# IBM/text-generation-inference

Measured on AMD Instinct MI355X. Metric: decode tokens/sec (Llama-7B int4 GPTQ, batch 32, ctx 1024) + p50 step latency, higher is better.
Workload: dtype f16

## Files before the change

### include/tgis_hip.h

```cpp
#ifndef TGIS_HIP_H
#define TGIS_HIP_H

#include <stdint.h>

#ifdef __cplusplus
extern "C" {
#endif

#define TGIS_OK 0
#define TGIS_EINVAL (-1)
#define TGIS_EHIP (-2)
#define TGIS_EUNSUPPORTED (-3)
#define TGIS_ENOMEM (-4)

#define TGIS_F16 0
#define TGIS_BF16 1

#define TGIS_KV_PAGE_TOKENS 32

#define TGIS_KV_MODEL 0
#define TGIS_KV_FP8_E4M3 1

const char* tgis_version(void);
const char* tgis_arch(void);
// ... 91 lines not shown
                             void* res_out, int64_t rows, int64_t hidden, float eps, int dtype, void* stream);
int tgis_layernorm2_residual_partial(const void* residual, const void* a, const float* a_slabs, int a_num_slabs,
                                     int64_t a_slab_ld, const void* a_bias, const void* b, const float* b_slabs,
                                     int b_num_slabs, int64_t b_slab_ld, const void* b_bias, const void* w1, const void* b1,
                                     const void* w2, const void* b2, void* y1, void* y2, void* res_out, int64_t rows,
                                     int64_t hidden, float eps, int dtype, void* stream);

int tgis_rope_kv_write(void* qkv, int64_t ld_qkv, const void* cos, const void* sin,
                       const int32_t* positions, const int32_t* slots, void* k_pool, void* v_pool,
                       int64_t T, int H, int Hkv, int D, int rot_dim, int dtype, void* stream);

int tgis_rope_kv_write_partial(const float* slabs, int num_slabs, int64_t slab_ld, const void* bias, void* qkv_out,
                               int64_t ld_qkv, const void* cos, const void* sin, const int32_t* positions,
                               const int32_t* slots, void* k_pool, void* v_pool, int64_t T, int H, int Hkv, int D,
                               int rot_dim, int dtype, void* stream);

int tgis_rope_kv_write_prefill(void* qkv, int64_t ld_qkv, const void* cos, const void* sin, const int32_t* positions,
                               const int32_t* cu_seqlens, const int32_t* block_tables, int64_t max_pages, void* k_pool,
                               void* v_pool, int64_t B, int64_t T, int64_t max_len, int H, int Hkv, int D, int rot_dim,
                               int dtype, void* stream);

int tgis_rope_kv_write_kv8(void* qkv, int64_t ld_qkv, const void* cos, const void* sin, const int32_t* positions,
                           const int32_t* slots, void* k_pool, void* v_pool, int64_t T, int H, int Hkv, int D, int rot_dim,
                           int dtype, void* stream, int kv_dtype, float k_scale, float v_scale);
int tgis_rope_kv_write_partial_kv8(const float* slabs, int num_slabs, int64_t slab_ld, const void* bias, void* qkv_out,
                                   int64_t ld_qkv, const void* cos, const void* sin, const int32_t* positions,
                                   const int32_t* slots, void* k_pool, void* v_pool, int64_t T, int H, int Hkv, int D,
                                   int rot_dim, int dtype, void* stream, int kv_dtype, float k_scale, float v_scale);
int tgis_rope_kv_write_prefill_kv8(void* qkv, int64_t ld_qkv, const void* cos, const void* sin, const int32_t* positions,
                                   const int32_t* cu_seqlens, const int32_t* block_tables, int64_t max_pages, void* k_pool,
                                   void* v_pool, int64_t B, int64_t T, int64_t max_len, int H, int Hkv, int D, int rot_dim,
                                   int dtype, void* stream, int kv_dtype, float k_scale, float v_scale);

int tgis_attn_num_splits(int64_t B, int Hkv, int H, int64_t max_q_len, int64_t max_ctx);
int64_t tgis_attn_workspace_bytes(int64_t total_q_tokens, int H, int Hkv, int D, int num_splits);
int tgis_attn_paged(const void* q, int64_t ld_q, const void* k_pool, const void* v_pool,
                    const int32_t* block_tables, int64_t max_pages, const int32_t* ctx_lens,
                    const int32_t* cu_seqlens_q, void* out, int64_t ld_out, int64_t B, int H, int Hkv, int D,
                    int64_t max_q_len, int64_t max_ctx, float scale, int dtype, int num_splits,
                    void* workspace, int64_t workspace_bytes, void* stream);
int tgis_attn_paged_kv8(const void* q, int64_t ld_q, const void* k_pool, const void* v_pool, const int32_t* block_tables,
                        int64_t max_pages, const int32_t* ctx_lens, const int32_t* cu_seqlens_q, void* out, int64_t ld_out,
                        int64_t B, int H, int Hkv, int D, int64_t max_q_len, int64_t max_ctx, float scale, int dtype,
                        int num_splits, void* workspace, int64_t workspace_bytes, void* stream, int kv_dtype,
                        float k_scale, float v_scale);

int tgis_act_mul(const void* gate_up, void* out, int64_t T, int64_t I, int act, int dtype, void* stream);
int tgis_gelu(const void* x, void* out, int64_t n, int tanh_approx, int dtype, void* stream);
int tgis_embedding(const int64_t* ids, const void* table, const int32_t* positions,
                   const void* pos_table, void* out, int64_t T, int64_t E, int64_t vocab_rows,
                   int64_t id_offset, int dtype, void* stream);
int tgis_decode_slots(const int32_t* positions, const int32_t* block_tables, int64_t max_pages,
                      int32_t* slots, int32_t* ctx_lens, int64_t B, void* stream);
int tgis_decode_advance(const int64_t* ids, int64_t* ids_copy, int64_t* position_ids, int64_t* all_input_ids,
                        int64_t ld_all, int32_t* cu_seqlens, const int32_t* cu_seqlens_q, int64_t* stage_ids,
                        int32_t* stage_positions, int64_t B, void* stream);

int64_t tgis_argmax_scratch_bytes(int64_t B);
int tgis_argmax_logprob(const void* logits, int64_t ld, int64_t B, int64_t V, int logits_f32, int dtype,
                        int64_t* ids_out, float* logprob_out, void* scratch, int64_t scratch_bytes, void* stream);

int tgis_warp_sample(const float* logits, int64_t ld_logits, float* scores, int64_t ld_scores, int64_t B,
                     int64_t V, const float* temperature, const int* top_k, const float* top_p_cut,
                     const float* typical_p, const float* rep_penalty, const int64_t* input_ids,
                     int64_t ld_ids, int64_t L, int64_t exclude_id, const float* eos_adjust, int64_t eos_id,
                     const int* do_sample, uint64_t* rng, int64_t* next_ids, float* next_logprob, float* lse,
                     void* stream);

#ifdef __cplusplus
}
#endif
#endif
```

### text-generation-inference_amd/csrc/norm.hip

```cpp
#include "common.h"
#include "dispatch.h"
#include "rowwise_plan.h"

namespace {

constexpr int MAX_HIDDEN = 16384;

template <int NT>
__device__ __forceinline__ float block_sum(float v, float* sh) {
    v = wave_sum(v);
    const int lane = threadIdx.x & 63, w = threadIdx.x >> 6;
    __syncthreads();
    if (lane == 0) sh[w] = v;
    __syncthreads();
    float t = 0.f;
#pragma unroll
    for (int k = 0; k < NT / 64; ++k) t += sh[k];
    return t;
}

template <typename T, bool RMS, bool PARTIAL, int NT>
__global__ __launch_bounds__(NT) void norm_kernel(const T* x, const T* residual,
                                                  const T* __restrict__ weight, const T* __restrict__ bias,
                                                  T* y, T* res_out, int hidden,
// ... 40 lines not shown
            V8 o;
            if (rr) {
#pragma unroll
                for (int e = 0; e < 8; ++e) v[it][e] = to_f32(a[e]) + to_f32(b[e]);
            } else {
#pragma unroll
                for (int e = 0; e < 8; ++e) v[it][e] = to_f32(a[e]);
            }
#pragma unroll
            for (int e = 0; e < 8; ++e) {
                o[e] = from_f32<T>(v[it][e]);
                s1 += v[it][e];
                s2 += v[it][e] * v[it][e];
            }
            if (res_out) st16(res_out + row * hidden + c * 8, o);
        }
    }
    float mean = 0.f, rstd;
    if (RMS) {
        float tot = block_sum<NT>(s2, sh);
        rstd = rsqrtf(tot / hidden + eps);
    } else {
        mean = block_sum<NT>(s1, sh) / hidden;
        float d2 = 0.f;
#pragma unroll
        for (int it = 0; it < MAXV; ++it) {
            int c = threadIdx.x + it * NT;
            if (c < nchunk) {
#pragma unroll
                for (int e = 0; e < 8; ++e) {
                    float d = v[it][e] - mean;
                    d2 += d * d;
                }
            }
        }
        float var = block_sum<NT>(d2, sh) / hidden;
        rstd = rsqrtf(var + eps);
    }
#pragma unroll
    for (int it = 0; it < MAXV; ++it) {
        int c = threadIdx.x + it * NT;
        if (c < nchunk) {
            const V8 wv = wvs[it];
            V8 o;
            if (bias) {
                const V8 bv = bvs[it];
#pragma unroll
                for (int e = 0; e < 8; ++e)
                    o[e] = from_f32<T>((v[it][e] - mean) * rstd * to_f32(wv[e]) + to_f32(bv[e]));
            } else {
#pragma unroll
                for (int e = 0; e < 8; ++e) o[e] = from_f32<T>((v[it][e] - mean) * rstd * to_f32(wv[e]));
            }
            st16(y + (y_frag ? xf_off(row, c * 8, hidden) : row * hidden + c * 8), o);
        }
    }
}

template <bool RMS>
static int launch_norm(const void* x, const void* residual, const void* weight, const void* bias, void* y,
                       void* res_out, int64_t rows, int64_t hidden, float eps, int dtype, void* stream,
                       const float* slabs = nullptr, int S = 0, int64_t slab_ld = 0, const void* xbias = nullptr,
                       int64_t ldy = 0) {
    TGIS_CHECK_ARG((x || slabs) && weight && y, "norm: null tensor");
    TGIS_CHECK_ARG(!slabs || (S >= 1 && slab_ld >= hidden && slab_ld % 4 == 0),
                   "norm: partial input needs a slab row stride >= hidden");
    TGIS_CHECK_ARG(hidden > 0 && hidden % 8 == 0 && hidden <= MAX_HIDDEN,
                   "norm: hidden (%ld) must be a multiple of 8 and <= %d", (long)hidden, MAX_HIDDEN);
    TGIS_CHECK_ARG(dtype == TGIS_F16 || dtype == TGIS_BF16, "norm: bad dtype");
    const int y_frag = ldy == TGIS_LD_FRAGMENTS;
    TGIS_CHECK_ARG(ldy == 0 || ldy == hidden || (y_frag && RMS && rows <= 64 && hidden % 64 == 0),
                   "norm: y is [rows, hidden] contiguous (ldy = 0 or hidden), or — RMSNorm, rows <= 64, hidden %% 64 == 0 — in "
                   "fragment order (ldy = TGIS_LD_FRAGMENTS)");
    if (rows == 0) return TGIS_OK;
    hipStream_t st = (hipStream_t)stream;
    TgisTimedScope timed(TGIS_OP_NORM, st);
    const bool wide = choose_norm(rows, hidden).nt == 512;
    return by_dtype(dtype, [&](auto t) {
        using T = type_of<decltype(t)>;
        return by_bool(slabs != nullptr, [&](auto partial) {
            return by_bool(wide, [&](auto w) {
                constexpr int NT = decltype(w)::value ? 512 : 256;
                hipLaunchKernelGGL((norm_kernel<T, RMS, decltype(partial)::value, NT>), dim3((unsigned)rows), dim3(NT), 0,
                                   st, (const T*)x, (const T*)residual, (const T*)weight, (const T*)bias, (T*)y,
                                   (T*)res_out, (int)hidden, eps, slabs, S, slab_ld, (const T*)xbias, y_frag);
                TGIS_CHECK_LAUNCH();
                return TGIS_OK;
            });
        });
    });
}

struct Addend {
    const void* x;
    const float* slabs;
    int S;
    int64_t slab_ld;
    const void* bias;
};

template <typename T>
__device__ __forceinline__ void add_addend(float (&v)[8], const Addend& ad, int64_t row, int hidden, int c) {
    using V8 = typename VecT<T>::x8;
    if (ad.slabs) {
        f32x4 lo, hi;
        sum_slabs8(ad.slabs + ((row >> 5) * ad.S * 32 + (row & 31)) * ad.slab_ld + c * 8, 32 * ad.slab_ld, ad.S, lo, hi);
// ... 87 lines not shown
                const V8 wb = ld16<V8>(w2 + c * 8), bb = ld16<V8>(b2 + c * 8);
#pragma unroll
                for (int e = 0; e < 8; ++e) o[e] = from_f32<T>(n[e] * to_f32(wb[e]) + to_f32(bb[e]));
                st16(y2 + row * hidden + c * 8, o);
            }
        }
    }
}

static int launch_layernorm2(const void* h, const Addend& A, const Addend& B, const void* w1, const void* b1,
                             const void* w2, const void* b2, void* y1, void* y2, void* res_out, int64_t rows,
                             int64_t hidden, float eps, int dtype, void* stream) {
    TGIS_CHECK_ARG(h && w1 && b1 && y1, "tgis_layernorm2_residual: null tensor");
    TGIS_CHECK_ARG(!y2 || (w2 && b2), "tgis_layernorm2_residual: y2 needs w2 and b2");
    TGIS_CHECK_ARG(!(A.x && A.slabs) && !(B.x && B.slabs), "tgis_layernorm2_residual: an addend is a tensor OR slabs");
    TGIS_CHECK_ARG((!A.slabs || (A.S >= 1 && A.slab_ld >= hidden && A.slab_ld % 4 == 0)) &&
                       (!B.slabs || (B.S >= 1 && B.slab_ld >= hidden && B.slab_ld % 4 == 0)),
                   "tgis_layernorm2_residual: slab input needs S >= 1 and a row stride >= hidden (multiple of 4)");
    TGIS_CHECK_ARG(hidden > 0 && hidden % 8 == 0 && hidden <= MAX_HIDDEN,
                   "tgis_layernorm2_residual: hidden (%ld) must be a multiple of 8 and <= %d", (long)hidden, MAX_HIDDEN);
    TGIS_CHECK_ARG(rows >= 0 && rows <= 2147483647LL, "tgis_layernorm2_residual: bad rows");
    TGIS_CHECK_ARG(dtype == TGIS_F16 || dtype == TGIS_BF16, "tgis_layernorm2_residual: bad dtype");
    if (rows == 0) return TGIS_OK;
    hipStream_t st = (hipStream_t)stream;
    TgisTimedScope timed(TGIS_OP_NORM, st);
    const bool wide = choose_norm(rows, hidden).nt == 512;
    return by_dtype(dtype, [&](auto t) {
        using T = type_of<decltype(t)>;
        return by_bool(wide, [&](auto w) {
            constexpr int NT = decltype(w)::value ? 512 : 256;
            hipLaunchKernelGGL((layernorm2_kernel<T, NT>), dim3((unsigned)rows), dim3(NT), 0, st, (const T*)h, A, B,
                               (const T*)w1, (const T*)b1, (const T*)w2, (const T*)b2, (T*)y1, (T*)y2, (T*)res_out,
                               (int)hidden, eps);
            TGIS_CHECK_LAUNCH();
            return TGIS_OK;
        });
    });
}

}

NormPlan choose_norm(int64_t rows, int64_t hidden) {
    const int nt = rows <= 64 && hidden >= 2048 ? 512 : 256;
    return {nt, (int)cdiv64(hidden / 8, nt)};
}

extern "C" int tgis_rmsnorm_residual(const void* x, const void* residual, const void* weight, void* y, int64_t ldy,
                                     void* res_out, int64_t rows, int64_t hidden, float eps, int dtype,
                                     void* stream) {
    return launch_norm<true>(x, residual, weight, nullptr, y, res_out, rows, hidden, eps, dtype, stream, nullptr, 0, 0,
                             nullptr, ldy);
}

extern "C" int tgis_rmsnorm_residual_partial(const float* slabs, int num_slabs, int64_t slab_ld, const void* bias,
                                             const void* residual, const void* weight, void* y, int64_t ldy, void* res_out,
                                             int64_t rows, int64_t hidden, float eps, int dtype, void* stream) {
    TGIS_CHECK_ARG(slabs, "tgis_rmsnorm_residual_partial: null slabs");
    return launch_norm<true>(nullptr, residual, weight, nullptr, y, res_out, rows, hidden, eps, dtype, stream, slabs,
                             num_slabs, slab_ld, bias, ldy);
}

extern "C" int tgis_layernorm_residual_partial(const float* slabs, int num_slabs, int64_t slab_ld, const void* xbias,
                                               const void* residual, const void* weight, const void* bias, void* y,
                                               void* res_out, int64_t rows, int64_t hidden, float eps, int dtype,
                                               void* stream) {
    TGIS_CHECK_ARG(slabs, "tgis_layernorm_residual_partial: null slabs");
    return launch_norm<false>(nullptr, residual, weight, bias, y, res_out, rows, hidden, eps, dtype, stream, slabs,
                              num_slabs, slab_ld, xbias);
}

extern "C" int tgis_layernorm_residual(const void* x, const void* residual, const void* weight,
                                       const void* bias, void* y, void* res_out, int64_t rows, int64_t hidden,
                                       float eps, int dtype, void* stream) {
    return launch_norm<false>(x, residual, weight, bias, y, res_out, rows, hidden, eps, dtype, stream);
}

extern "C" int tgis_layernorm2_residual(const void* residual, const void* a, const void* a_bias, const void* b,
                                        const void* b_bias, const void* w1, const void* b1, const void* w2, const void* b2,
                                        void* y1, void* y2, void* res_out, int64_t rows, int64_t hidden, float eps,
                                        int dtype, void* stream) {
    const Addend A{a, nullptr, 0, 0, a_bias}, B{b, nullptr, 0, 0, b_bias};
    return launch_layernorm2(residual, A, B, w1, b1, w2, b2, y1, y2, res_out, rows, hidden, eps, dtype, stream);
}

extern "C" int tgis_layernorm2_residual_partial(const void* residual, const void* a, const float* a_slabs, int a_num_slabs,
                                                int64_t a_slab_ld, const void* a_bias, const void* b, const float* b_slabs,
                                                int b_num_slabs, int64_t b_slab_ld, const void* b_bias, const void* w1,
                                                const void* b1, const void* w2, const void* b2, void* y1, void* y2,
                                                void* res_out, int64_t rows, int64_t hidden, float eps, int dtype,
                                                void* stream) {
    const Addend A{a, a_slabs, a_num_slabs, a_slab_ld, a_bias}, B{b, b_slabs, b_num_slabs, b_slab_ld, b_bias};
    return launch_layernorm2(residual, A, B, w1, b1, w2, b2, y1, y2, res_out, rows, hidden, eps, dtype, stream);
}
```

### text-generation-inference_amd/tgis_amd/models/custom_modeling/flash_common.py

```python
from dataclasses import dataclass
from typing import Optional

import torch

from tgis_amd import native
from tgis_amd.utils.layers import workspace


@dataclass
class KVArgs:
    cache: "object"
    block_tables: torch.Tensor
    ctx_lens: Optional[torch.Tensor]
    slots: Optional[torch.Tensor]
    max_q_len: int
    max_ctx: int
    num_splits: int = 1
    fresh_prefill: bool = False


def layer_pools(kv: KVArgs, layer_id: int):
    cache = kv.cache
    scales = {"kv_scales": cache.scales(layer_id)} if cache.is_fp8 else {}
    return cache.k_pool(layer_id), cache.v_pool(layer_id), scales


def write_kv(qkv, kv: KVArgs, layer_id: int, H: int, Hkv: int, D: int, rot_dim: int, cos, sin, position_ids, cu_seqlens_q):
    k_pool, v_pool, scales = layer_pools(kv, layer_id)
    if kv.fresh_prefill and not isinstance(qkv, native.Partial):
        return native.rope_kv_write_prefill(qkv, cos, sin, position_ids, cu_seqlens_q, kv.block_tables, k_pool, v_pool,
                                            kv.max_q_len, H, Hkv, D, rot_dim, **scales)
    return native.rope_kv_write(qkv, cos, sin, position_ids, kv.slots, k_pool, v_pool, H, Hkv, D, rot_dim, **scales)


def attend(qkv, kv: KVArgs, layer_id: int, H: int, Hkv: int, D: int, scale: float, cu_seqlens_q, frag_out: bool = False):
    k_pool, v_pool, scales = layer_pools(kv, layer_id)
    T = qkv.shape[0]
    if frag_out:
        attn_output = native.FragAct.empty(T, H * D, qkv.device)
    else:
        attn_output = torch.empty((T, H * D), dtype=qkv.dtype, device=qkv.device)
    ws = None
    if kv.num_splits > 1:
        ws = workspace(qkv.device)
        ws.ensure(native.attn_workspace_bytes(T, H, Hkv, D, kv.num_splits))
    native.attn_paged(qkv, qkv.stride(0), k_pool, v_pool, kv.block_tables, kv.ctx_lens, cu_seqlens_q, attn_output,
                      kv.block_tables.shape[0], H, Hkv, D, kv.max_q_len, kv.max_ctx, scale, kv.num_splits, ws, **scales)
    return attn_output


class FastLayerNorm:
    def __init__(self, prefix, weights, eps):
        self.weight = weights.get_tensor(f"{prefix}.weight").contiguous()
        self.bias = weights.get_tensor(f"{prefix}.bias").contiguous()
        self.eps = eps

    def forward(self, hidden_states, residual=None):
        return native.layernorm_residual(hidden_states, residual, self.weight, self.bias, self.eps)

    __call__ = forward


def grow_max_positions(config, max_positions: int, max_s: int) -> int:
    if max_s <= max_positions:
        return max_positions
    declared = min(int(getattr(config, "max_position_embeddings", 0) or 0), 1 << 17)
    return max(max_s, 2 * max_positions, declared, 2048)


class FlashForCausalLM:

# ... 20 lines not shown
```

### text-generation-inference_amd/tgis_amd/models/custom_modeling/flash_llama_modeling.py

```python
from tgis_amd import native
from tgis_amd.models.custom_modeling.flash_common import (
    FlashForCausalLM,
    KVArgs,
    attend,
    grow_max_positions,
    layer_pools,
    write_kv,
)
from tgis_amd.utils.layers import (
    PositionRotaryEmbedding,
    TensorParallelColumnLinear,
    TensorParallelEmbedding,
    TensorParallelHead,
    TensorParallelRowLinear,
)


class LlamaConfig:

    def __init__(self, vocab_size=32000, hidden_size=4096, intermediate_size=11008, num_hidden_layers=32,
                 num_attention_heads=32, num_key_value_heads=None, hidden_act="silu", max_position_embeddings=2048,
                 rms_norm_eps=1e-6, rope_scaling=None, rope_theta=10000.0, attention_bias=False, mlp_bias=False,
                 pad_token_id=None, bos_token_id=1, eos_token_id=2, tie_word_embeddings=False, quantize=None,
                 **kwargs):
# ... 95 lines not shown
        return write_kv(qkv, kv, layer_id, H, Hkv, D, D, cos, sin, position_ids, cu_seqlens_q)

    def attend(self, qkv, cu_seqlens_q, layer_id: int, kv: KVArgs):
        return attend(qkv, kv, layer_id, self.num_heads, self.num_key_value_heads, self.head_size, self.softmax_scale,
                      cu_seqlens_q, frag_out=frag_rows(self.o_proj.linear, qkv.shape[0], kv))

    def forward(self, hidden_states, cos, sin, position_ids, cu_seqlens_q, layer_id: int, kv: KVArgs):
        qkv = self.project_qkv(hidden_states, cos, sin, position_ids, cu_seqlens_q, layer_id, kv)
        attn_output = self.attend(qkv, cu_seqlens_q, layer_id, kv)
        return self.o_proj(attn_output, partial=True)

    __call__ = forward


class LlamaMLP:
    def __init__(self, prefix, config, weights):
        if config.hidden_act != "silu":
            raise NotImplementedError(f"hidden_act {config.hidden_act}: only silu is wired into the fused kernel")
        self.gate_up_proj = TensorParallelColumnLinear.load_multi(
            config, prefixes=[f"{prefix}.gate_proj", f"{prefix}.up_proj"], weights=weights, dim=0,
            bias=config.mlp_bias)
        self.down_proj = TensorParallelRowLinear.load(config, prefix=f"{prefix}.down_proj", weights=weights,
                                                      bias=config.mlp_bias)
        self.intermediate_size = config.intermediate_size // weights.process_group.size()
        self.fused_epilogue = hasattr(self.gate_up_proj.linear, "gate_up") and self.intermediate_size % 16 == 0
        if self.fused_epilogue:
            self.gate_up_proj.linear.gate_up = True

    def forward(self, hidden_states):
        if self.fused_epilogue:
            if isinstance(hidden_states, native.FragAct):
                rows = hidden_states.shape[0]
                act = self.gate_up_proj(hidden_states, out_frag=self.down_proj.linear.wants_fragments(rows))
                return self.down_proj(act, partial=True)
            act = self.gate_up_proj(hidden_states)
            return self.down_proj(act, partial=True)
        gate_up_states = self.gate_up_proj(hidden_states)
        return self.down_proj(gate_up_states, act=1, partial=True)

    __call__ = forward


class FlashLlamaLayer:
    def __init__(self, layer_id, config, weights):
        prefix = f"model.layers.{layer_id}"
        self.layer_id = layer_id
        self.self_attn = FlashLlamaAttention(prefix=f"{prefix}.self_attn", config=config, weights=weights)
        self.mlp = LlamaMLP(prefix=f"{prefix}.mlp", config=config, weights=weights)
        self.input_layernorm = LlamaRMSNorm(prefix=f"{prefix}.input_layernorm", weights=weights,
                                            eps=config.rms_norm_eps)
        self.post_attention_layernorm = LlamaRMSNorm(prefix=f"{prefix}.post_attention_layernorm", weights=weights,
                                                     eps=config.rms_norm_eps)

    def forward(self, hidden_states, residual, cos, sin, position_ids, cu_seqlens_q, kv: KVArgs):
        rows = hidden_states.shape[0]
        att = self.self_attn
        qkv_frag = (kv.slots is not None and cos.shape[1] * 2 == att.head_size
                    and frag_rows(att.query_key_value.linear, rows, kv, act=3))
        normed_hidden_states, res = self.input_layernorm(hidden_states, residual, frag=qkv_frag)
        attn_output = att(normed_hidden_states, cos, sin, position_ids, cu_seqlens_q, self.layer_id, kv)
        mlp_frag = self.mlp.fused_epilogue and frag_rows(self.mlp.gate_up_proj.linear, rows, kv, act=2)
        normed_attn_res_output, attn_res = self.post_attention_layernorm(attn_output, res, frag=mlp_frag)
        mlp_output = self.mlp(normed_attn_res_output)
        return mlp_output, attn_res

    __call__ = forward


class FlashLlamaModel:
    def __init__(self, config, weights):
        self.config = config
        process_group = weights.process_group
        self.tp_rank = process_group.rank()
        self.tp_world_size = process_group.size()
        self.embed_tokens = TensorParallelEmbedding(prefix="model.embed_tokens", weights=weights)
        self.layers = [FlashLlamaLayer(i, config, weights) for i in range(config.num_hidden_layers)]
        self.norm = LlamaRMSNorm(prefix="model.norm", weights=weights, eps=config.rms_norm_eps)
        self.head_size = self.layers[0].self_attn.head_size
        self.num_heads = self.layers[0].self_attn.num_heads
        self.num_key_value_heads = config.num_key_value_heads // process_group.size()
        self.max_positions = 0

    def rope_tables(self, dtype, device, max_s: int):
        self.max_positions = grow_max_positions(self.config, self.max_positions, max_s)
        return self.layers[0].self_attn.rotary_emb.tables(dtype, device, self.max_positions)

    def forward(self, input_ids, position_ids, cu_seqlens_q, max_s, inputs_embeds, kv: KVArgs):
        hidden_states = inputs_embeds if inputs_embeds is not None else self.embed_tokens(input_ids)
        cos, sin = self.rope_tables(hidden_states.dtype, hidden_states.device, max_s)
        residual = None
        for layer in self.layers:
            hidden_states, residual = layer(hidden_states, residual, cos, sin, position_ids, cu_seqlens_q, kv)
        hidden_states, _ = self.norm(hidden_states, residual)
        return hidden_states

    __call__ = forward


class FlashLlamaForCausalLM(FlashForCausalLM):
    def __init__(self, config, weights):
        self.config = config
        self.model = FlashLlamaModel(config, weights)
        self.lm_head = TensorParallelHead.load(config, prefix="lm_head", weights=weights)
        self.gptq_linears = []
        for layer in self.model.layers:
            for lin in (layer.self_attn.query_key_value.linear, layer.self_attn.o_proj.linear,
                        layer.mlp.gate_up_proj.linear, layer.mlp.down_proj.linear):
                if hasattr(lin, "post_init"):
                    self.gptq_linears.append(lin)

    def get_input_embeddings(self):
        return self.model.embed_tokens
```

### text-generation-inference_amd/tgis_amd/models/flash_causal_lm.py

```python
import logging
import os
import time
from collections import OrderedDict, deque
from dataclasses import dataclass
from operator import itemgetter
from typing import Any, List, Optional, Tuple, Type, Union

import numpy as np
import torch

from tgis_amd import native
from tgis_amd.models.custom_modeling.flash_common import KVArgs
from tgis_amd.models.model import Model
from tgis_amd.models.types import Batch, GenerateError
from tgis_amd.pb import generate_pb2
from tgis_amd.utils.graph_segments import SegmentedGraph, no_gc_during_capture
from tgis_amd.utils.kv_cache import (KV_CACHE_DTYPES, PAGE, PagedKVCache, kv_pool_dtype, pages_for_budget,
                                     parse_kv_cache_dtype)
from tgis_amd.utils.token_types import InputTokens, TokenInfo
from tgis_amd.utils.tokens import HeterogeneousNextTokenChooser, get_input_tokens_info, get_token_info

logger = logging.getLogger(__name__)

USE_GRAPHS = os.getenv("TGIS_DISABLE_GRAPHS", "false").lower() not in ("1", "true")
# ... 242 lines not shown

FRESH_PREFILL_KV = os.getenv("TGIS_PREFILL_KV", "true").lower() not in ("0", "false")


GRAPH_BUCKETS = os.getenv("TGIS_GRAPH_BUCKETS", "true").lower() not in ("0", "false")


def graph_bucket(B: int) -> int:
    if not GRAPH_BUCKETS:
        return B
    if B <= 8:
        return 1 << (B - 1).bit_length()
    return (B + 7) // 8 * 8


class _DecodeGraph:

    def __init__(self, lm: "FlashCausalLM", B: int, width: int):
        dev = lm.device
        self.rows = B
        self.active = 0
        self.input_ids = torch.zeros(B, dtype=torch.int64, device=dev)
        self.positions = torch.zeros(B, dtype=torch.int32, device=dev)
        self.block_tables = torch.full((B, width), lm.kv_cache.null_page, dtype=torch.int32, device=dev)
        self.slots = torch.zeros(B, dtype=torch.int32, device=dev)
        self.ctx = torch.ones(B, dtype=torch.int32, device=dev)
        self.cu_q = torch.arange(B + 1, dtype=torch.int32, device=dev)
        self.max_ctx = width * PAGE
        self.num_splits = native.attn_num_splits(B, lm.num_kv_heads, lm.num_heads, 1, self.max_ctx)
        self.lm = lm
        self.graph = None
        self.logits = self.ids = self.logprobs = None
        self.out_buf = torch.zeros(B * 12, dtype=torch.uint8, device=dev)
        self.ids_buf = self.out_buf[:B * 8].view(torch.int64)
        self.lps_buf = self.out_buf[B * 8:].view(torch.float32)
        self.argmax_scratch = native.argmax_scratch(B, dev)
        self.host_buf = torch.zeros(B * 12, dtype=torch.uint8).pin_memory()
        self.host_ready = torch.cuda.Event()
        self.staged_ids = self.staged_pos = self.staged_bt = None

    def fetch_greedy(self):
        self.host_buf.copy_(self.out_buf, non_blocking=True)
        self.host_ready.record()
        return self._read_host

    def _read_host(self, want_logprobs: bool):
        self.host_ready.synchronize()
        B = self.ids_buf.numel()
        ids = self.host_buf[:B * 8].view(torch.int64).tolist()
        return ids, (self.host_buf[B * 8:].view(torch.float32).tolist() if want_logprobs else None)

    def _step(self):
        lm = self.lm
        native.decode_slots(self.positions, self.block_tables, self.slots, self.ctx)
        kv = KVArgs(cache=lm.kv_cache, block_tables=self.block_tables, ctx_lens=self.ctx, slots=self.slots,
                    max_q_len=1, max_ctx=self.max_ctx, num_splits=self.num_splits)
        logits = lm.model.forward(self.input_ids, self.positions, self.cu_q, self.max_ctx, None, kv)
        ids, lps = native.argmax_logprob(logits, ids_out=self.ids_buf, logprob_out=self.lps_buf, scratch=self.argmax_scratch)
        return logits, ids, lps

    def run(self, input_ids, position_ids, block_tables):
        n = input_ids.numel()
        if n < self.active:
            self.positions[n:self.active].zero_()
            self.input_ids[n:self.active].zero_()
            self.block_tables[n:self.active].fill_(self.lm.kv_cache.null_page)
        self.active = n
        if input_ids is not self.staged_ids or position_ids is not self.staged_pos:
            self.input_ids[:n].copy_(input_ids, non_blocking=True)
            self.positions[:n].copy_(position_ids, non_blocking=True)
        if block_tables is not self.staged_bt:
            self.block_tables[:n].copy_(block_tables, non_blocking=True)
            self.staged_bt = block_tables
        self.staged_ids = self.staged_pos = None
        logits, ids, lps = self._run()
        return (logits, ids, lps) if n == self.rows else (logits[:n], ids[:n], lps[:n])

    def _run(self):
        if not self.lm.use_graphs:
            return self._step()
        if self.graph is None:
            t_capture = time.perf_counter()
            self._step()
            torch.cuda.current_stream().synchronize()
            g = None
            if self.lm.resolve_graph_mode() == "full":
                g = torch.cuda.CUDAGraph()
                kw = {"capture_error_mode": "thread_local"} if self.lm.tp_world > 1 else {}
                ok = True
                try:
                    with no_gc_during_capture(), torch.cuda.graph(g, pool=self.lm.graph_pool, **kw):
                        self.logits, self.ids, self.logprobs = self._step()
                except Exception as exc:
                    if self.lm.tp_world == 1:
                        raise
                    logger.warning("capturing the tensor-parallel step with RCCL inside failed (%s)", exc)
                    native.clear_error()
                    ok = False
                if self.lm.tp_world > 1 and not self.lm.all_ranks_agree(ok):
                    self.lm.graph_mode = "segments"
                    g = None
            if g is None:
                if not any(d.graph is not None for d in self.lm._graphs.values()):
                    self.lm.graph_pool = torch.cuda.graph_pool_handle()
                g = SegmentedGraph(self.lm.device, pool=self.lm.graph_pool)
                try:
                    self.logits, self.ids, self.logprobs = g.record(self._step)
                except Exception as exc:
                    logger.warning("segmented capture of the decode step failed (%s); running eagerly", exc)
# ... 292 lines not shown
```

### text-generation-inference_amd/tgis_amd/native.py

```python
import ctypes
import os
from typing import Optional

import torch

_HERE = os.path.dirname(os.path.abspath(__file__))
LIB_PATH = os.getenv("TGIS_HIP_LIB") or os.path.join(os.path.dirname(_HERE), "lib", "libtgis_hip.so")

F16, BF16 = 0, 1
KV_PAGE_TOKENS = 32

OP_GPTQ_GEMM, OP_ATTN, OP_DENSE_GEMM, OP_NORM, OP_ROPE_KV, OP_ACT, OP_SAMPLE = range(7)

_c_i64 = ctypes.c_int64
_c_int = ctypes.c_int
_c_f = ctypes.c_float
_vp = ctypes.c_void_p
_KV8_ARGS = [_c_int, _c_f, _c_f]


SIGNATURES = {
    "tgis_version": (ctypes.c_char_p, []),
    "tgis_arch": (ctypes.c_char_p, []),
    "tgis_clear_error": (None, []),
# ... 13 lines not shown
                                            ctypes.POINTER(_c_int), ctypes.POINTER(_c_i64), _vp]),
    "tgis_gptq_dequant_f16": (_c_int, [_vp, _vp, _c_i64, _c_i64, _c_i64, _c_int, _vp]),
    "tgis_dense_gemm_rope": (_c_int, [_vp, _c_i64, _vp, _vp, _vp, _vp, _vp, _vp, _vp, _c_i64, _vp, _vp, _c_i64, _c_i64, _c_i64,
                                      _c_i64, _c_i64, _c_i64, _c_int, _vp]),
    "tgis_dense_gemm_rope_kv8": (_c_int, [_vp, _c_i64, _vp, _vp, _vp, _vp, _vp, _vp, _vp, _c_i64, _vp, _vp, _c_i64, _c_i64,
                                          _c_i64, _c_i64, _c_i64, _c_i64, _c_int, _vp] + _KV8_ARGS),
    "tgis_gptq_rope_ok": (_c_int, [_c_i64, _c_i64, _c_i64, _c_i64, _c_int, _c_i64]),
    "tgis_gptq_fragments_ok": (_c_int, [_c_i64, _c_i64, _c_i64, _c_i64, _c_int, _c_int]),
    "tgis_dense_rope_ok": (_c_int, [_c_i64, _c_i64, _c_i64, _c_i64]),
    "tgis_gptq_gemm_rope_f16": (_c_int, [_vp, _c_i64, _vp, _vp, _vp, _vp, _vp, _vp, _vp, _c_i64, _vp, _vp, _c_i64, _c_i64,
                                         _c_i64, _c_i64, _c_i64, _c_i64, _c_i64, _vp]),
    "tgis_gptq_gemm_rope_f16_kv8": (_c_int, [_vp, _c_i64, _vp, _vp, _vp, _vp, _vp, _vp, _vp, _c_i64, _vp, _vp, _c_i64,
                                             _c_i64, _c_i64, _c_i64, _c_i64, _c_i64, _c_i64, _vp] + _KV8_ARGS),
    "tgis_dense_prepared_bytes": (_c_i64, [_c_i64, _c_i64]),
    "tgis_dense_prepare": (_c_int, [_vp, _c_i64, _c_i64, _c_int, _c_int, _vp, _vp]),
    "tgis_dense_gemm_workspace_bytes": (_c_i64, [_c_i64, _c_i64, _c_i64]),
    "tgis_dense_gemm": (_c_int, [_vp, _c_i64, _vp, _vp, _vp, _c_i64, _c_i64, _c_i64, _c_i64, _c_int, _c_int,
                                 _c_int, _vp, _c_i64, _vp]),
    "tgis_dense_gemm_partial_bytes": (_c_i64, [_c_i64, _c_i64, _c_i64]),
    "tgis_dense_gemm_partial": (_c_int, [_vp, _c_i64, _vp, _c_i64, _c_i64, _c_i64, _c_int, _c_int, _vp, _c_i64,
                                         ctypes.POINTER(_c_int), ctypes.POINTER(_c_i64), _vp]),
    "tgis_rmsnorm_residual": (_c_int, [_vp, _vp, _vp, _vp, _c_i64, _vp, _c_i64, _c_i64, _c_f, _c_int, _vp]),
    "tgis_rmsnorm_residual_partial": (_c_int, [_vp, _c_int, _c_i64, _vp, _vp, _vp, _vp, _c_i64, _vp, _c_i64, _c_i64, _c_f,
                                               _c_int, _vp]),
    "tgis_layernorm_residual": (_c_int, [_vp, _vp, _vp, _vp, _vp, _vp, _c_i64, _c_i64, _c_f, _c_int, _vp]),
    "tgis_layernorm_residual_partial": (_c_int, [_vp, _c_int, _c_i64, _vp, _vp, _vp, _vp, _vp, _vp, _c_i64, _c_i64,
                                                 _c_f, _c_int, _vp]),
    "tgis_layernorm2_residual": (_c_int, [_vp, _vp, _vp, _vp, _vp, _vp, _vp, _vp, _vp, _vp, _vp, _vp, _c_i64, _c_i64,
                                          _c_f, _c_int, _vp]),
    "tgis_layernorm2_residual_partial": (_c_int, [_vp, _vp, _vp, _c_int, _c_i64, _vp, _vp, _vp, _c_int, _c_i64, _vp, _vp,
                                                  _vp, _vp, _vp, _vp, _vp, _vp, _c_i64, _c_i64, _c_f, _c_int, _vp]),
    "tgis_rope_kv_write": (_c_int, [_vp, _c_i64, _vp, _vp, _vp, _vp, _vp, _vp, _c_i64, _c_int, _c_int, _c_int,
                                    _c_int, _c_int, _vp]),
    "tgis_rope_kv_write_partial": (_c_int, [_vp, _c_int, _c_i64, _vp, _vp, _c_i64, _vp, _vp, _vp, _vp, _vp, _vp, _c_i64,
                                            _c_int, _c_int, _c_int, _c_int, _c_int, _vp]),
    "tgis_rope_kv_write_prefill": (_c_int, [_vp, _c_i64, _vp, _vp, _vp, _vp, _vp, _c_i64, _vp, _vp, _c_i64, _c_i64, _c_i64,
                                            _c_int, _c_int, _c_int, _c_int, _c_int, _vp]),
    "tgis_rope_kv_write_kv8": (_c_int, [_vp, _c_i64, _vp, _vp, _vp, _vp, _vp, _vp, _c_i64, _c_int, _c_int, _c_int,
                                        _c_int, _c_int, _vp] + _KV8_ARGS),
    "tgis_rope_kv_write_partial_kv8": (_c_int, [_vp, _c_int, _c_i64, _vp, _vp, _c_i64, _vp, _vp, _vp, _vp, _vp, _vp, _c_i64,
                                                _c_int, _c_int, _c_int, _c_int, _c_int, _vp] + _KV8_ARGS),
    "tgis_rope_kv_write_prefill_kv8": (_c_int, [_vp, _c_i64, _vp, _vp, _vp, _vp, _vp, _c_i64, _vp, _vp, _c_i64, _c_i64,
                                                _c_i64, _c_int, _c_int, _c_int, _c_int, _c_int, _vp] + _KV8_ARGS),
    "tgis_attn_num_splits": (_c_int, [_c_i64, _c_int, _c_int, _c_i64, _c_i64]),
    "tgis_attn_workspace_bytes": (_c_i64, [_c_i64, _c_int, _c_int, _c_int, _c_int]),
    "tgis_attn_paged": (_c_int, [_vp, _c_i64, _vp, _vp, _vp, _c_i64, _vp, _vp, _vp, _c_i64, _c_i64, _c_int, _c_int,
                                 _c_int, _c_i64, _c_i64, _c_f, _c_int, _c_int, _vp, _c_i64, _vp]),
    "tgis_attn_paged_kv8": (_c_int, [_vp, _c_i64, _vp, _vp, _vp, _c_i64, _vp, _vp, _vp, _c_i64, _c_i64, _c_int, _c_int,
                                     _c_int, _c_i64, _c_i64, _c_f, _c_int, _c_int, _vp, _c_i64, _vp] + _KV8_ARGS),
    "tgis_act_mul": (_c_int, [_vp, _vp, _c_i64, _c_i64, _c_int, _c_int, _vp]),
    "tgis_gelu": (_c_int, [_vp, _vp, _c_i64, _c_int, _c_int, _vp]),
    "tgis_embedding": (_c_int, [_vp, _vp, _vp, _vp, _vp, _c_i64, _c_i64, _c_i64, _c_i64, _c_int, _vp]),
    "tgis_decode_slots": (_c_int, [_vp, _vp, _c_i64, _vp, _vp, _c_i64, _vp]),
    "tgis_decode_advance": (_c_int, [_vp, _vp, _vp, _vp, _c_i64, _vp, _vp, _vp, _vp, _c_i64, _vp]),
    "tgis_argmax_logprob": (_c_int, [_vp, _c_i64, _c_i64, _c_i64, _c_int, _c_int, _vp, _vp, _vp, _c_i64, _vp]),
    "tgis_argmax_scratch_bytes": (_c_i64, [_c_i64]),
    "tgis_warp_sample": (_c_int, [_vp, _c_i64, _vp, _c_i64, _c_i64, _c_i64, _vp, _vp, _vp, _vp, _vp, _vp, _c_i64,
                                  _c_i64, _c_i64, _vp, _c_i64, _vp, _vp, _vp, _vp, _vp, _vp]),
}

_lib = None


class TgisHipError(RuntimeError):
    pass


def load_library(path: Optional[str] = None) -> ctypes.CDLL:
    global _lib
    if _lib is not None and path is None:
        return _lib
    p = path or LIB_PATH
    if not os.path.exists(p):
        raise TgisHipError(
            f"{p} not found: build the HIP extension first (python -c 'import __graft_entry__ as g; g.build()')"
        )
    lib = ctypes.CDLL(p)
    for name, (res, args) in SIGNATURES.items():
        fn = getattr(lib, name)
        fn.restype = res
        fn.argtypes = args
    if path is None:
        _lib = lib
    return lib


def _check(rc: int, what: str):
    if rc != 0:
        msg = load_library().tgis_last_error().decode()
        raise TgisHipError(f"{what} failed (code {rc}): {msg}")


KV_MODEL, KV_FP8_E4M3 = 0, 1
KV8_DTYPES = (torch.uint8, torch.float8_e4m3fn)


def kv_is8(pool: Optional[torch.Tensor]) -> bool:
    return pool is not None and pool.dtype in KV8_DTYPES


def _call_kv(name: str, args: tuple, k_pool, v_pool, kv_scales) -> None:
    if kv_is8(k_pool):
        assert kv_is8(v_pool) and k_pool.dtype == v_pool.dtype, "k and v pools must both hold e4m3 codes"
        k_scale, v_scale = (1.0, 1.0) if kv_scales is None else kv_scales
        name += "_kv8"
        args += (KV_FP8_E4M3, float(k_scale), float(v_scale))
# ... 484 lines not shown
    if isinstance(out, FragAct):
        assert max_q_len == 1 and out.K == H * D and out.M == B
        optr, ldo = _ptr(out.buf), LD_FRAGMENTS
    else:
        assert out.is_contiguous()
        optr, ldo = _ptr(out), H * D
    wptr, wbytes = (ws.ptr, ws.nbytes) if ws is not None else (None, 0)
    args = (_ptr(q), ld_q, _ptr(k_pool), _ptr(v_pool), _ptr(block_tables), block_tables.shape[1], _ptr(ctx_lens),
            _ptr(cu_seqlens_q), optr, ldo, B, H, Hkv, D, max_q_len, max_ctx, float(scale), dtype_code(q.dtype), num_splits,
            wptr, wbytes, _stream())
    _call_kv("tgis_attn_paged", args, k_pool, v_pool, kv_scales)
    return out


def act_mul(gate_up, I: int, out=None):
    T = gate_up.shape[0]
    assert gate_up.is_contiguous() and gate_up.shape[1] == 2 * I
    if out is None:
        out = torch.empty((T, I), dtype=gate_up.dtype, device=gate_up.device)
    _check(load_library().tgis_act_mul(_ptr(gate_up), _ptr(out), T, I, 1, dtype_code(gate_up.dtype), _stream()),
           "tgis_act_mul")
    return out


def gelu(x, tanh_approx: bool, out=None):
    assert x.is_contiguous()
    if out is None:
        out = torch.empty_like(x)
    _check(load_library().tgis_gelu(_ptr(x), _ptr(out), x.numel(), int(tanh_approx), dtype_code(x.dtype), _stream()),
           "tgis_gelu")
    return out


def embedding(ids, table, positions=None, pos_table=None, id_offset: int = 0, out=None):
    assert ids.dtype == torch.int64 and ids.is_contiguous() and table.is_contiguous()
    T = ids.numel()
    E = table.shape[1]
    if out is None:
        out = torch.empty((T, E), dtype=table.dtype, device=table.device)
    _check(
        load_library().tgis_embedding(_ptr(ids), _ptr(table), _ptr(positions), _ptr(pos_table), _ptr(out), T, E,
                                      table.shape[0], id_offset, dtype_code(table.dtype), _stream()),
        "tgis_embedding")
    return out


def decode_slots(positions, block_tables, slots, ctx_lens):
    B = positions.numel()
    _check(
        load_library().tgis_decode_slots(_ptr(positions), _ptr(block_tables), block_tables.shape[1], _ptr(slots),
                                         _ptr(ctx_lens), B, _stream()), "tgis_decode_slots")


def decode_advance(ids, position_ids, all_input_ids=None, cu_seqlens=None, cu_seqlens_q=None, stage_ids=None,
                   stage_positions=None):
    B = ids.numel()
    assert ids.dtype == torch.int64 and position_ids.dtype == torch.int64 and position_ids.numel() == B
    assert ids.is_contiguous() and position_ids.is_contiguous()
    out = torch.empty_like(ids)
    ld = 0
    if all_input_ids is not None:
        assert all_input_ids.dtype == torch.int64 and all_input_ids.stride(1) == 1 and all_input_ids.shape[0] >= B
        ld = all_input_ids.stride(0)
    if cu_seqlens is not None:
        assert cu_seqlens.dtype == torch.int32 and cu_seqlens_q.dtype == torch.int32
        assert cu_seqlens.numel() == B + 1 and cu_seqlens_q.numel() == B + 1
    if stage_ids is not None:
        assert stage_ids.dtype == torch.int64 and stage_ids.numel() == B
    if stage_positions is not None:
        assert stage_positions.dtype == torch.int32 and stage_positions.numel() == B
    _check(
        load_library().tgis_decode_advance(_ptr(ids), _ptr(out), _ptr(position_ids), _ptr(all_input_ids), ld,
                                           _ptr(cu_seqlens), _ptr(cu_seqlens_q), _ptr(stage_ids), _ptr(stage_positions),
                                           B, _stream()), "tgis_decode_advance")
    return out


def argmax_scratch(B: int, device) -> torch.Tensor:
    return torch.empty(max(16, load_library().tgis_argmax_scratch_bytes(B)), dtype=torch.uint8, device=device)


def argmax_logprob(logits, ids_out=None, logprob_out=None, scratch=None):
    assert logits.dim() == 2 and logits.stride(1) == 1
    B, V = logits.shape
    if ids_out is None:
        ids_out = torch.empty(B, dtype=torch.int64, device=logits.device)
    if logprob_out is None:
        logprob_out = torch.empty(B, dtype=torch.float32, device=logits.device)
    f32 = logits.dtype == torch.float32
    _check(
        load_library().tgis_argmax_logprob(_ptr(logits), logits.stride(0), B, V, int(f32),
                                           0 if f32 else dtype_code(logits.dtype), _ptr(ids_out),
                                           _ptr(logprob_out), _ptr(scratch), scratch.numel() if scratch is not None else 0,
                                           _stream()), "tgis_argmax_logprob")
    return ids_out, logprob_out


def warp_sample(logits, temperature=None, top_k=None, top_p_cut=None, typical_p=None, rep_penalty=None,
                input_ids=None, exclude_id: int = -1, eos_adjust=None, eos_id: int = -1, do_sample=None, rng=None):
    assert logits.dim() == 2 and logits.dtype == torch.float32 and logits.stride(1) == 1
    B, V = logits.shape
    dev = logits.device
    for t, dt in ((temperature, torch.float32), (top_k, torch.int32), (top_p_cut, torch.float32),
                  (typical_p, torch.float32), (rep_penalty, torch.float32), (do_sample, torch.int32)):
        assert t is None or (t.dtype == dt and t.numel() == B and t.is_contiguous() and t.device == dev)
    assert rng is None or (rng.dtype == torch.int64 and rng.shape == (B, 2) and rng.is_contiguous())
# ... 18 lines not shown
```

Measured before the change: 7255.

## Fuse embedding lookup, decode slot computation and first RMSNorm into one kernel

Adds a kernel that, per decode row, gathers the embedding row, computes the KV slot and context length, writes the residual, and applies the first layer's input RMSNorm (optionally in fragment layout). The decode step skips the separate decode_slots launch, and layer 0 receives the pre-normed input. This removes two kernel launches and one round-trip of the hidden states per step. It only applies when tensor parallel size is 1, and slots are now written inside the model's forward pass rather than before it.

```diff
diff --git a/include/tgis_hip.h b/include/tgis_hip.h
--- a/include/tgis_hip.h
+++ b/include/tgis_hip.h
@@ -167,6 +167,10 @@
                    int64_t id_offset, int dtype, void* stream);
 int tgis_decode_slots(const int32_t* positions, const int32_t* block_tables, int64_t max_pages,
                       int32_t* slots, int32_t* ctx_lens, int64_t B, void* stream);
+int tgis_embed_slots_rmsnorm(const int64_t* ids, const void* table, int64_t vocab_rows, int64_t id_offset,
+                             const int32_t* positions, const int32_t* block_tables, int64_t max_pages, int32_t* slots,
+                             int32_t* ctx_lens, const void* weight, void* y, int64_t ldy, void* res_out, int64_t rows,
+                             int64_t hidden, float eps, int dtype, void* stream);
 int tgis_decode_advance(const int64_t* ids, int64_t* ids_copy, int64_t* position_ids, int64_t* all_input_ids,
                         int64_t ld_all, int32_t* cu_seqlens, const int32_t* cu_seqlens_q, int64_t* stage_ids,
                         int32_t* stage_positions, int64_t B, void* stream);
diff --git a/text-generation-inference_amd/csrc/norm.hip b/text-generation-inference_amd/csrc/norm.hip
--- a/text-generation-inference_amd/csrc/norm.hip
+++ b/text-generation-inference_amd/csrc/norm.hip
@@ -116,6 +116,63 @@
 #pragma unroll
                 for (int e = 0; e < 8; ++e) o[e] = from_f32<T>((v[it][e] - mean) * rstd * to_f32(wv[e]));
             }
+            st16(y + (y_frag ? xf_off(row, c * 8, hidden) : row * hidden + c * 8), o);
+        }
+    }
+}
+
+template <typename T, int NT>
+__global__ __launch_bounds__(NT) void embed_slots_norm_kernel(const int64_t* __restrict__ ids, const T* __restrict__ table,
+                                                              int64_t vocab_rows, int64_t id_offset,
+                                                              const int32_t* __restrict__ positions,
+                                                              const int32_t* __restrict__ bt, int64_t max_pages,
+                                                              int32_t* __restrict__ slots, int32_t* __restrict__ ctx,
+                                                              const T* __restrict__ weight, T* __restrict__ y,
+                                                              T* __restrict__ res_out, int hidden, float eps, int y_frag) {
+    using V8 = typename VecT<T>::x8;
+    constexpr int MAXV = MAX_HIDDEN / (NT * 8);
+    __shared__ float sh[NT / 64];
+    const int64_t row = blockIdx.x;
+    const int64_t id = ids[row] - id_offset;
+    const bool valid = id >= 0 && id < vocab_rows;
+    const T* xr = table + (valid ? id : 0) * hidden;
+    if (threadIdx.x == 0) {
+        const int pos = positions[row];
+        const int page = bt[row * max_pages + (pos >> 5)];
+        slots[row] = page * TGIS_KV_PAGE_TOKENS + (pos & 31);
+        ctx[row] = pos + 1;
+    }
+    float v[MAXV][8];
+    V8 wvs[MAXV];
+    const int nchunk = hidden >> 3;
+    float s2 = 0.f;
+#pragma unroll
+    for (int it = 0; it < MAXV; ++it) {
+        int c = threadIdx.x + it * NT;
+        if (c < nchunk) {
+            wvs[it] = ld16<V8>(weight + c * 8);
+            V8 a;
+#pragma unroll
+            for (int e = 0; e < 8; ++e) a[e] = (T)0.f;
+            if (valid) a = ld16<V8>(xr + c * 8);
+#pragma unroll
+            for (int e = 0; e < 8; ++e) {
+                v[it][e] = to_f32(a[e]);
+                s2 += v[it][e] * v[it][e];
+            }
+            st16(res_out + row * hidden + c * 8, a);
+        }
+    }
+    const float tot = block_sum<NT>(s2, sh);
+    const float mean = 0.f, rstd = rsqrtf(tot / hidden + eps);
+#pragma unroll
+    for (int it = 0; it < MAXV; ++it) {
+        int c = threadIdx.x + it * NT;
+        if (c < nchunk) {
+            const V8 wv = wvs[it];
+            V8 o;
+#pragma unroll
+            for (int e = 0; e < 8; ++e) o[e] = from_f32<T>((v[it][e] - mean) * rstd * to_f32(wv[e]));
             st16(y + (y_frag ? xf_off(row, c * 8, hidden) : row * hidden + c * 8), o);
         }
     }
@@ -309,6 +366,38 @@
                              nullptr, ldy);
 }
 
+extern "C" int tgis_embed_slots_rmsnorm(const int64_t* ids, const void* table, int64_t vocab_rows, int64_t id_offset,
+                                        const int32_t* positions, const int32_t* block_tables, int64_t max_pages,
+                                        int32_t* slots, int32_t* ctx_lens, const void* weight, void* y, int64_t ldy,
+                                        void* res_out, int64_t rows, int64_t hidden, float eps, int dtype, void* stream) {
+    TGIS_CHECK_ARG(ids && table && positions && block_tables && slots && ctx_lens && weight && y && res_out,
+                   "tgis_embed_slots_rmsnorm: null tensor");
+    TGIS_CHECK_ARG(max_pages > 0 && vocab_rows > 0 && rows >= 0 && rows <= 2147483647LL,
+                   "tgis_embed_slots_rmsnorm: bad arguments");
+    TGIS_CHECK_ARG(hidden > 0 && hidden % 8 == 0 && hidden <= MAX_HIDDEN,
+                   "tgis_embed_slots_rmsnorm: hidden (%ld) must be a multiple of 8 and <= %d", (long)hidden, MAX_HIDDEN);
+    TGIS_CHECK_ARG(dtype == TGIS_F16 || dtype == TGIS_BF16, "tgis_embed_slots_rmsnorm: bad dtype");
+    const int y_frag = ldy == TGIS_LD_FRAGMENTS;
+    TGIS_CHECK_ARG(ldy == 0 || ldy == hidden || (y_frag && rows <= 64 && hidden % 64 == 0),
+                   "tgis_embed_slots_rmsnorm: y is [rows, hidden] contiguous (ldy = 0 or hidden), or — rows <= 64, hidden %% 64 "
+                   "== 0 — in fragment order (ldy = TGIS_LD_FRAGMENTS)");
+    if (rows == 0) return TGIS_OK;
+    hipStream_t st = (hipStream_t)stream;
+    TgisTimedScope timed(TGIS_OP_NORM, st);
+    const bool wide = choose_norm(rows, hidden).nt == 512;
+    return by_dtype(dtype, [&](auto t) {
+        using T = type_of<decltype(t)>;
+        return by_bool(wide, [&](auto w) {
+            constexpr int NT = decltype(w)::value ? 512 : 256;
+            hipLaunchKernelGGL((embed_slots_norm_kernel<T, NT>), dim3((unsigned)rows), dim3(NT), 0, st, ids, (const T*)table,
+                               vocab_rows, id_offset, positions, block_tables, max_pages, slots, ctx_lens, (const T*)weight,
+                               (T*)y, (T*)res_out, (int)hidden, eps, y_frag);
+            TGIS_CHECK_LAUNCH();
+            return TGIS_OK;
+        });
+    });
+}
+
 extern "C" int tgis_rmsnorm_residual_partial(const float* slabs, int num_slabs, int64_t slab_ld, const void* bias,
                                              const void* residual, const void* weight, void* y, int64_t ldy, void* res_out,
                                              int64_t rows, int64_t hidden, float eps, int dtype, void* stream) {
diff --git a/text-generation-inference_amd/tgis_amd/models/custom_modeling/flash_common.py b/text-generation-inference_amd/tgis_amd/models/custom_modeling/flash_common.py
--- a/text-generation-inference_amd/tgis_amd/models/custom_modeling/flash_common.py
+++ b/text-generation-inference_amd/tgis_amd/models/custom_modeling/flash_common.py
@@ -17,6 +17,7 @@
     max_ctx: int
     num_splits: int = 1
     fresh_prefill: bool = False
+    slots_pending: bool = False
 
 
 def layer_pools(kv: KVArgs, layer_id: int):
diff --git a/text-generation-inference_amd/tgis_amd/models/custom_modeling/flash_llama_modeling.py b/text-generation-inference_amd/tgis_amd/models/custom_modeling/flash_llama_modeling.py
--- a/text-generation-inference_amd/tgis_amd/models/custom_modeling/flash_llama_modeling.py
+++ b/text-generation-inference_amd/tgis_amd/models/custom_modeling/flash_llama_modeling.py
@@ -171,12 +171,20 @@
         self.post_attention_layernorm = LlamaRMSNorm(prefix=f"{prefix}.post_attention_layernorm", weights=weights,
                                                      eps=config.rms_norm_eps)
 
-    def forward(self, hidden_states, residual, cos, sin, position_ids, cu_seqlens_q, kv: KVArgs):
-        rows = hidden_states.shape[0]
+    def qkv_frag(self, rows: int, cos, kv: KVArgs) -> bool:
         att = self.self_attn
-        qkv_frag = (kv.slots is not None and cos.shape[1] * 2 == att.head_size
-                    and frag_rows(att.query_key_value.linear, rows, kv, act=3))
-        normed_hidden_states, res = self.input_layernorm(hidden_states, residual, frag=qkv_frag)
+        return (kv.slots is not None and cos.shape[1] * 2 == att.head_size
+                and frag_rows(att.query_key_value.linear, rows, kv, act=3))
+
+    def forward(self, hidden_states, residual, cos, sin, position_ids, cu_seqlens_q, kv: KVArgs, normed=None):
+        att = self.self_attn
+        if normed is None:
+            rows = hidden_states.shape[0]
+            normed_hidden_states, res = self.input_layernorm(hidden_states, residual,
+                                                             frag=self.qkv_frag(rows, cos, kv))
+        else:
+            normed_hidden_states, res = normed
+            rows = res.shape[0]
         attn_output = att(normed_hidden_states, cos, sin, position_ids, cu_seqlens_q, self.layer_id, kv)
         mlp_frag = self.mlp.fused_epilogue and frag_rows(self.mlp.gate_up_proj.linear, rows, kv, act=2)
         normed_attn_res_output, attn_res = self.post_attention_layernorm(attn_output, res, frag=mlp_frag)
@@ -199,16 +207,29 @@
         self.num_heads = self.layers[0].self_attn.num_heads
         self.num_key_value_heads = config.num_key_value_heads // process_group.size()
         self.max_positions = 0
+        self.fuses_decode_slots = self.tp_world_size == 1
 
     def rope_tables(self, dtype, device, max_s: int):
         self.max_positions = grow_max_positions(self.config, self.max_positions, max_s)
         return self.layers[0].self_attn.rotary_emb.tables(dtype, device, self.max_positions)
 
     def forward(self, input_ids, position_ids, cu_seqlens_q, max_s, inputs_embeds, kv: KVArgs):
-        hidden_states = inputs_embeds if inputs_embeds is not None else self.embed_tokens(input_ids)
-        cos, sin = self.rope_tables(hidden_states.dtype, hidden_states.device, max_s)
-        residual = None
-        for layer in self.layers:
+        if kv.slots_pending:
+            assert self.fuses_decode_slots and inputs_embeds is None
+            emb, first = self.embed_tokens, self.layers[0]
+            cos, sin = self.rope_tables(emb.weight.dtype, emb.weight.device, max_s)
+            norm = first.input_layernorm
+            normed = native.embed_slots_rmsnorm(input_ids, emb.weight, position_ids, kv.block_tables, kv.slots, kv.ctx_lens,
+                                                norm.weight, norm.variance_epsilon, id_offset=emb.min_id,
+                                                frag=first.qkv_frag(input_ids.numel(), cos, kv))
+            hidden_states, residual = first(None, None, cos, sin, position_ids, cu_seqlens_q, kv, normed=normed)
+            rest = self.layers[1:]
+        else:
+            hidden_states = inputs_embeds if inputs_embeds is not None else self.embed_tokens(input_ids)
+            cos, sin = self.rope_tables(hidden_states.dtype, hidden_states.device, max_s)
+            residual = None
+            rest = self.layers
+        for layer in rest:
             hidden_states, residual = layer(hidden_states, residual, cos, sin, position_ids, cu_seqlens_q, kv)
         hidden_states, _ = self.norm(hidden_states, residual)
         return hidden_states
diff --git a/text-generation-inference_amd/tgis_amd/models/flash_causal_lm.py b/text-generation-inference_amd/tgis_amd/models/flash_causal_lm.py
--- a/text-generation-inference_amd/tgis_amd/models/flash_causal_lm.py
+++ b/text-generation-inference_amd/tgis_amd/models/flash_causal_lm.py
@@ -318,9 +318,11 @@
 
     def _step(self):
         lm = self.lm
-        native.decode_slots(self.positions, self.block_tables, self.slots, self.ctx)
+        fused = getattr(lm.model.model, "fuses_decode_slots", False)
+        if not fused:
+            native.decode_slots(self.positions, self.block_tables, self.slots, self.ctx)
         kv = KVArgs(cache=lm.kv_cache, block_tables=self.block_tables, ctx_lens=self.ctx, slots=self.slots,
-                    max_q_len=1, max_ctx=self.max_ctx, num_splits=self.num_splits)
+                    max_q_len=1, max_ctx=self.max_ctx, num_splits=self.num_splits, slots_pending=fused)
         logits = lm.model.forward(self.input_ids, self.positions, self.cu_q, self.max_ctx, None, kv)
         ids, lps = native.argmax_logprob(logits, ids_out=self.ids_buf, logprob_out=self.lps_buf, scratch=self.argmax_scratch)
         return logits, ids, lps
diff --git a/text-generation-inference_amd/tgis_amd/native.py b/text-generation-inference_amd/tgis_amd/native.py
--- a/text-generation-inference_amd/tgis_amd/native.py
+++ b/text-generation-inference_amd/tgis_amd/native.py
@@ -89,6 +89,8 @@
     "tgis_gelu": (_c_int, [_vp, _vp, _c_i64, _c_int, _c_int, _vp]),
     "tgis_embedding": (_c_int, [_vp, _vp, _vp, _vp, _vp, _c_i64, _c_i64, _c_i64, _c_i64, _c_int, _vp]),
     "tgis_decode_slots": (_c_int, [_vp, _vp, _c_i64, _vp, _vp, _c_i64, _vp]),
+    "tgis_embed_slots_rmsnorm": (_c_int, [_vp, _vp, _c_i64, _c_i64, _vp, _vp, _c_i64, _vp, _vp, _vp, _vp, _c_i64, _vp,
+                                          _c_i64, _c_i64, _c_f, _c_int, _vp]),
     "tgis_decode_advance": (_c_int, [_vp, _vp, _vp, _vp, _c_i64, _vp, _vp, _vp, _vp, _c_i64, _vp]),
     "tgis_argmax_logprob": (_c_int, [_vp, _c_i64, _c_i64, _c_i64, _c_int, _c_int, _vp, _vp, _vp, _c_i64, _vp]),
     "tgis_argmax_scratch_bytes": (_c_i64, [_c_i64]),
@@ -679,6 +681,28 @@
                                          _ptr(ctx_lens), B, _stream()), "tgis_decode_slots")
 
 
+def embed_slots_rmsnorm(ids, table, positions, block_tables, slots, ctx_lens, weight, eps: float, id_offset: int = 0,
+                        frag: bool = False):
+    assert ids.dtype == torch.int64 and ids.is_contiguous() and table.is_contiguous() and weight.dtype == table.dtype
+    assert positions.dtype == torch.int32 and block_tables.dtype == torch.int32 and block_tables.is_contiguous()
+    rows, hidden = ids.numel(), table.shape[1]
+    assert positions.numel() == rows and block_tables.shape[0] == rows and slots.numel() == rows and ctx_lens.numel() == rows
+    res = torch.empty((rows, hidden), dtype=table.dtype, device=table.device)
+    yf = None
+    if frag:
+        assert rows <= 64 and hidden % 64 == 0 and table.dtype == torch.float16
+        yf = FragAct.empty(rows, hidden, table.device)
+        y, ldy = yf.buf, LD_FRAGMENTS
+    else:
+        y, ldy = torch.empty_like(res), hidden
+    _check(
+        load_library().tgis_embed_slots_rmsnorm(_ptr(ids), _ptr(table), table.shape[0], id_offset, _ptr(positions),
+                                                _ptr(block_tables), block_tables.shape[1], _ptr(slots), _ptr(ctx_lens),
+                                                _ptr(weight), _ptr(y), ldy, _ptr(res), rows, hidden, float(eps),
+                                                dtype_code(table.dtype), _stream()), "tgis_embed_slots_rmsnorm")
+    return (yf if frag else y), res
+
+
 def decode_advance(ids, position_ids, all_input_ids=None, cu_seqlens=None, cu_seqlens_q=None, stage_ids=None,
                    stage_positions=None):
     B = ids.numel()
```

New measurement: 7271 (median of 4 runs). No clear change (+0.2%).
